# chy980959830/Multi-Modal-Retrieval-System-Image-Search-and-Data-Governance

Hardware: AMD Instinct MI355X
Metric: images/sec encode + Mqueries/sec top-10 over 1M×512 gallery, 1→8 MI355X (higher is better)
Workload: dtype bf16; 1 GPU; ViT-B/32 bf16 encode batch 256/GPU + top-10 of 256 queries over 1000000x512 bf16 gallery rows/GPU (BASELINE configs[1]); encode_batch_per_gpu=256, gallery_rows_per_gpu=1000000, gallery_rows_total=1000000, queries=256, k=10, embed_dim=512, parallelism=single GPU, launch=single process, steps_in_flight=2, weights=seeded random init (no checkpoint reachable offline)

## Files before the change

include/mmr.h:

```cpp
#ifndef MMR_H
#define MMR_H

#include <stddef.h>
#include <stdint.h>

#ifdef __cplusplus
extern "C" {
#endif

typedef enum { MMR_F32 = 0, MMR_BF16 = 1 } mmr_dtype;

enum {
    MMR_OK = 0,
    MMR_EIO = -5,
    MMR_EINVAL = -22,
    MMR_ENOSPC = -28,
    MMR_ENOTSUP = -95
};

const char *mmr_last_error(void);
int mmr_version(void);


size_t mmr_search_workspace_bytes(int64_t N, int E, int Q, int k);
// ... 109 lines not shown

typedef enum {
    MMR_P_PATCH_W = 0, MMR_P_CLS, MMR_P_POS, MMR_P_LN_PRE_W, MMR_P_LN_PRE_B,
    MMR_P_LN1_W, MMR_P_LN1_B, MMR_P_QKV_W, MMR_P_QKV_B, MMR_P_OUT_W, MMR_P_OUT_B,
    MMR_P_LN2_W, MMR_P_LN2_B, MMR_P_FC1_W, MMR_P_FC1_B, MMR_P_FC2_W, MMR_P_FC2_B,
    MMR_P_LN_FINAL_W, MMR_P_LN_FINAL_B, MMR_P_PROJ, MMR_P_TOK_EMB,
    MMR_P_TYPE_EMB,
    MMR_P_POOL_W,
    MMR_P_POOL_B,
    MMR_P_PROJ_B,
    MMR_P_QKV_C,
    MMR_P_FC1_C,
    MMR_P_COUNT
} mmr_param;

size_t mmr_tower_weights_bytes(const mmr_tower_cfg *cfg);
int mmr_tower_param_span(const mmr_tower_cfg *cfg, int param, int layer, size_t *offset, size_t *bytes);

typedef struct mmr_tower mmr_tower;

#define MMR_STATUS_BAD_TOKEN_ID 1

int mmr_tower_set_shared_chip(mmr_tower *t, int shared);
int mmr_tower_create(const mmr_tower_cfg *cfg, const void *weights, size_t weights_bytes, mmr_tower **out);
void mmr_tower_destroy(mmr_tower *t);
size_t mmr_tower_workspace_bytes(const mmr_tower *t, int batch);

int mmr_vit_encode_image(mmr_tower *t, const void *pixels, mmr_dtype in_dtype, int B, void *out,
                         mmr_dtype out_dtype, int normalize, void *workspace, size_t workspace_bytes,
                         void *stream);

int mmr_text_encode(mmr_tower *t, const int32_t *ids, int N, void *out, mmr_dtype out_dtype, int normalize,
                    void *workspace, size_t workspace_bytes, void *stream);

size_t mmr_bert_workspace_bytes(const mmr_tower *t, int N, int T);
int mmr_bert_forward(mmr_tower *t, const int32_t *ids, int N, int T, void *out, mmr_dtype out_dtype, int normalize,
                     int tap_after, float *tap, void *workspace, size_t workspace_bytes, void *stream);
int mmr_bert_forward_masked(mmr_tower *t, const int32_t *ids, const int32_t *token_type_ids,
                            const int32_t *attention_mask, int N, int T, void *out, mmr_dtype out_dtype, int normalize,
                            int tap_after, float *tap, void *workspace, size_t workspace_bytes, void *stream);

int mmr_tower_forward(mmr_tower *t, const void *input, mmr_dtype in_dtype, int B, void *out,
                      mmr_dtype out_dtype, int normalize, int tap_after, float *tap, void *workspace,
                      size_t workspace_bytes, void *stream);


// ... 44 lines not shown
```

multi-modal-retrieval-system-image-search-and-data-governance_amd/_lib.py:

```python
import ctypes
import os

import torch

_HERE = os.path.dirname(os.path.abspath(__file__))
LIB_PATH = os.environ.get("MMR_LIB") or os.path.join(_HERE, "csrc", "libmmr_hip.so")

MMR_F32, MMR_BF16 = 0, 1
_ERRNAMES = {-5: "EIO", -22: "EINVAL", -28: "ENOSPC", -95: "ENOTSUP"}


class MMRError(RuntimeError):
    def __init__(self, code, msg):
        super().__init__(f"libmmr_hip: {_ERRNAMES.get(code, code)}: {msg}")
        self.code = code


class TowerCfg(ctypes.Structure):
    _fields_ = [(n, ctypes.c_int) for n in
                ("kind", "width", "layers", "heads", "mlp", "tokens", "embed_dim", "image_size", "patch", "vocab")]
    _fields_.append(("ln_eps", ctypes.c_float))
    _fields_.append(("fold_ln", ctypes.c_int))


# ... 85 lines not shown
    L.mmr_tip_adapter_logits.argtypes = [vp, vp, vp, vp, i32, i64, i32, i32, i32, f32, f32, vp, vp, vp]
    L.mmr_preprocess_image.restype = i32
    L.mmr_preprocess_image.argtypes = [vp, i32, i32, i32, i32, i32, vp, vp, i32, vp, vp, i32, f32, f32, f32, f32, f32,
                                       f32, vp, vp, i32, vp, vp]
    L.mmr_preprocess_batch.restype = i32
    L.mmr_preprocess_batch.argtypes = [vp, i32, i32, i32, f32, f32, f32, f32, f32, f32, vp, i32, vp]
    L.mmr_preprocess_batch_ex.restype = i32
    L.mmr_preprocess_batch_ex.argtypes = [vp, i32, i32, i32, i32, f32, f32, f32, f32, f32, f32, vp, i32, vp]
    L.mmr_prof_enable.restype = i32
    L.mmr_prof_enable.argtypes = [i32, i32]
    L.mmr_prof_read.restype = i32
    L.mmr_prof_read.argtypes = [i32, ctypes.POINTER(ctypes.c_double), ctypes.POINTER(ctypes.c_longlong),
                                ctypes.POINTER(ctypes.c_longlong)]
    if hasattr(L, "mmr_tower_create"):
        cfgp = ctypes.POINTER(TowerCfg)
        L.mmr_tower_weights_bytes.restype = sz
        L.mmr_tower_weights_bytes.argtypes = [cfgp]
        L.mmr_tower_param_span.restype = i32
        L.mmr_tower_param_span.argtypes = [cfgp, i32, i32, ctypes.POINTER(sz), ctypes.POINTER(sz)]
        L.mmr_tower_create.restype = i32
        L.mmr_tower_create.argtypes = [cfgp, vp, sz, ctypes.POINTER(vp)]
        L.mmr_tower_set_shared_chip.restype = i32
        L.mmr_tower_set_shared_chip.argtypes = [vp, i32]
        L.mmr_tower_destroy.restype = None
        L.mmr_tower_destroy.argtypes = [vp]
        L.mmr_tower_workspace_bytes.restype = sz
        L.mmr_tower_workspace_bytes.argtypes = [vp, i32]
        L.mmr_vit_encode_image.restype = i32
        L.mmr_vit_encode_image.argtypes = [vp, vp, i32, i32, vp, i32, i32, vp, sz, vp]
        L.mmr_text_encode.restype = i32
        L.mmr_text_encode.argtypes = [vp, vp, i32, vp, i32, i32, vp, sz, vp]
        L.mmr_tower_forward.restype = i32
        L.mmr_tower_forward.argtypes = [vp, vp, i32, i32, vp, i32, i32, i32, vp, vp, sz, vp]
        L.mmr_bert_workspace_bytes.restype = sz
        L.mmr_bert_workspace_bytes.argtypes = [vp, i32, i32]
        L.mmr_bert_forward.restype = i32
        L.mmr_bert_forward.argtypes = [vp, vp, i32, i32, vp, i32, i32, i32, vp, vp, sz, vp]
        L.mmr_bert_forward_masked.restype = i32
        L.mmr_bert_forward_masked.argtypes = [vp, vp, vp, vp, i32, i32, vp, i32, i32, i32, vp, vp, sz, vp]
        L.mmr_debug_attention_masked.restype = i32
        L.mmr_debug_attention_masked.argtypes = [vp, vp, i32, i32, i32, vp, vp]
        L.mmr_debug_gemm.restype = i32
        L.mmr_debug_gemm.argtypes = [i32, vp, vp, i32, i32, i32, vp, vp, vp]
        L.mmr_debug_gemm_fold.restype = i32
        L.mmr_debug_gemm_fold.argtypes = [i32, vp, vp, i32, i32, i32, vp, vp, vp, vp, f32, f32, vp, vp, vp]
        L.mmr_debug_layernorm.restype = i32
# ... 44 lines not shown
```

multi-modal-retrieval-system-image-search-and-data-governance_amd/clip.py:

```python
import contextlib
import ctypes
import os
from typing import Dict, List, Optional, Union

import torch

from . import _lib
from .config import ClipConfig, TowerConfig, available_models, get_config
from .weights import make_clip_weights

_CONTEXT = 77
CLIP_MEAN = (0.48145466, 0.4578275, 0.40821073)
CLIP_STD = (0.26862954, 0.26130258, 0.27577711)


def _fold_ln_default() -> bool:
    return os.environ.get("MMR_FOLD_LN", "0") == "1"


def _tower_cfg_struct(t: TowerConfig, fold_ln: bool = False) -> _lib.TowerCfg:
    return _lib.TowerCfg(kind=0 if t.kind == "vision" else 1, width=t.width, layers=t.layers, heads=t.heads,
                         mlp=t.mlp, tokens=t.tokens, embed_dim=t.embed_dim, image_size=t.image_size,
                         patch=t.patch, vocab=t.vocab, ln_eps=t.ln_eps, fold_ln=int(bool(fold_ln)))

# ... 66 lines not shown
                put(pid, i, lw[name], bf)

        self.blob = blob.to(device)
        handle = ctypes.c_void_p()
        _lib.check(self.L.mmr_tower_create(ctypes.byref(self.c), self.blob.data_ptr(), self.blob.numel(),
                                           ctypes.byref(handle)))
        self.handle = handle
        self._lanes = {}

    def __del__(self):
        h, self.handle = getattr(self, "handle", None), None
        if h:
            try:
                self.L.mmr_tower_destroy(h)
            except Exception:
                pass

    @property
    def _ws(self):
        return self._lanes.get(0)

    def set_shared_chip(self, shared: bool) -> None:
        _lib.check(self.L.mmr_tower_set_shared_chip(self.handle, int(bool(shared))))

    def workspace(self, batch: int, lane: int = 0) -> torch.Tensor:
        need = self.L.mmr_tower_workspace_bytes(self.handle, batch)
        ws = self._lanes.get(lane)
        if ws is None or ws.numel() < need:
            ws = torch.empty(need, dtype=torch.uint8, device=self.device)
            self._lanes[lane] = ws
        return ws

    def status_word(self, lane: int = 0) -> int:
        ws = self._lanes.get(lane)
        return 0 if ws is None else int(ws[:4].view(torch.int32)[0])

    def forward(self, inp: torch.Tensor, out_dtype: torch.dtype, normalize: bool, tap_after: int = -1,
                tap: Optional[torch.Tensor] = None, out: Optional[torch.Tensor] = None, lane: int = 0) -> torch.Tensor:
        B = inp.shape[0]
        if out is None:
            out = torch.empty(B, self.cfg.embed_dim, dtype=out_dtype, device=self.device)
        elif (tuple(out.shape) != (B, self.cfg.embed_dim) or out.dtype != out_dtype or not out.is_contiguous()
              or out.device != self.device):
            raise ValueError(f"out must be a contiguous {out_dtype} [{B},{self.cfg.embed_dim}] tensor on {self.device}")
        if B == 0:
            return out
# ... 321 lines not shown
```

multi-modal-retrieval-system-image-search-and-data-governance_amd/csrc/tower.hip:

```cpp
#include "mmr_common.h"

#include <new>

namespace mmr {
enum { EPI_BIAS_BF16 = 0, EPI_BIAS_GELU_BF16 = 1, EPI_BIAS_RESID_F32 = 2, EPI_STORE_F32 = 3,
       EPI_BIAS_F32 = 4, EPI_BIAS_GELU_ERF_BF16 = 5, EPI_BIAS_TANH_BF16 = 6, EPI_LNFOLD_BF16 = 7, EPI_LNFOLD_GELU_BF16 = 8,
       EPI_RESID_STATS_F32 = 9 };
int launch_gemm(int epi, const bf16_t *A, const bf16_t *W, int M, int N, int K, const float *bias, void *out, hipStream_t st);
int launch_gemm_patch32(const bf16_t *pix, int B, int S, const bf16_t *W, int M, int N, float *out, hipStream_t st);
int launch_gemm_aux(int epi, const bf16_t *A, const bf16_t *W, int M, int N, int K, const float *bias, void *out, const GemmAux &aux, hipStream_t st);
void gemm_set_shared_chip_hint(bool on);
int launch_im2col(const void *px, mmr_dtype dt, bf16_t *ap, int B, int S, int P, int G, int K, int Kpad, hipStream_t st);
int launch_embed_vision(const float *pe, const float *cls, const float *pos, const float *lw, const float *lb, float *h, int B, int T, int d, float eps, bf16_t *xb, float2 *stats, int32_t *status, hipStream_t st);
int launch_embed_text(const int32_t *ids, const bf16_t *tok, const float *pos, float *h, int Nb, int T, int d, int vocab, bf16_t *xb, float2 *stats, int32_t *status, hipStream_t st);
int launch_layernorm(const float *h, const float *w, const float *b, bf16_t *x, int64_t rows, int d, float eps, hipStream_t st);
int launch_pool_ln(const float *h, const int32_t *ids, const float *w, const float *b, bf16_t *xc, int Nb, int T, int d, float eps, hipStream_t st);
int launch_finish(const float *feat, void *out, mmr_dtype odt, int Nb, int E, int normalize, hipStream_t st);
int launch_embed_bert(const int32_t *ids, const bf16_t *tok, const float *pos, const float *type0, const float *lw, const float *lb, float *h, bf16_t *x, int Nb, int T, int d, int vocab, float eps, const int32_t *types, int32_t *status, hipStream_t st);
int launch_layernorm_inplace(float *h, const float *w, const float *b, bf16_t *x, int64_t rows, int d, float eps, hipStream_t st);
int launch_gather_first_rows(const bf16_t *x, bf16_t *xc, int Nb, int T, int d, hipStream_t st);
int launch_attention(const bf16_t *qkv, bf16_t *o, int Bn, int T, int heads, int d, int causal, const int32_t *kmask, hipStream_t st);

static inline int round_up(int x, int a) { return (x + a - 1) / a * a; }

static int patch_k(const mmr_tower_cfg &c) { return 3 * c.patch * c.patch; }
static int patch_kpad(const mmr_tower_cfg &c) { return round_up(patch_k(c), 64); }

static const char *validate_cfg(const mmr_tower_cfg *c)
{
    if (!c) return "null config";
    if (c->kind < 0 || c->kind > 2) return "kind must be 0 (vision), 1 (text) or 2 (BERT text)";
    if (c->width != 128 && c->width != 512 && c->width != 768 && c->width != 1024) return "width must be 128, 512, 768 or 1024";
    if (c->heads * 64 != c->width) return "heads must equal width / 64 (head dim 64)";
    if (c->layers < 1 || c->layers > 64) return "layers outside [1,64]";
    if (c->mlp < 128 || c->mlp % 128) return "mlp must be a positive multiple of 128";
    if (c->embed_dim < 128 || c->embed_dim % 128) return "embed_dim must be a positive multiple of 128";
    if (c->tokens < 1 || c->tokens > 608) return "tokens outside [1,608]";
    if (!(c->ln_eps > 0.f)) return "ln_eps must be > 0";
    if (c->fold_ln != 0 && c->fold_ln != 1) return "fold_ln must be 0 or 1";
    if (c->fold_ln && c->kind == 2) return "fold_ln is for pre-LN (CLIP) towers; BERT towers are post-LN";
    if (c->kind == 0) {
        if (c->patch < 1 || c->image_size < c->patch || c->image_size % c->patch) return "image_size must be a multiple of patch";
        const int g = c->image_size / c->patch;
        if (c->tokens != 1 + g * g) return "vision tokens must equal 1 + (image_size/patch)^2";
// ... 51 lines not shown
    put(L.layer0[MMR_P_FC1_B], m * 4);
    put(L.layer0[MMR_P_FC2_W], d * m * 2);
    put(L.layer0[MMR_P_FC2_B], d * 4);
    if (c.fold_ln) {
        put(L.layer0[MMR_P_QKV_C], 3 * d * 4);
        put(L.layer0[MMR_P_FC1_C], m * 4);
    }
    L.layer_stride = off - l0;
    L.total = l0 + L.layer_stride * c.layers;
    return L;
}

static bool is_layer_param(int p) { return (p >= MMR_P_LN1_W && p <= MMR_P_FC2_B) || p == MMR_P_QKV_C || p == MMR_P_FC1_C; }

}

using namespace mmr;

struct mmr_tower {
    mmr_tower_cfg cfg;
    Layout lay;
    const char *w;
    bool shared_chip = false;
    template <typename T> const T *g(int p) const { return reinterpret_cast<const T *>(w + lay.global[p].off); }
    template <typename T> const T *l(int p, int layer) const {
        return reinterpret_cast<const T *>(w + lay.layer0[p].off + (size_t)layer * lay.layer_stride);
    }
};

extern "C" size_t mmr_tower_weights_bytes(const mmr_tower_cfg *cfg)
{
    if (validate_cfg(cfg)) return 0;
    return make_layout(*cfg).total;
}

extern "C" int mmr_tower_param_span(const mmr_tower_cfg *cfg, int param, int layer, size_t *offset, size_t *bytes)
{
    const char *why = validate_cfg(cfg);
    MMR_CHECK_ARG(!why, "mmr_tower_param_span: %s", why);
    MMR_CHECK_ARG(param >= 0 && param < MMR_P_COUNT && offset && bytes, "mmr_tower_param_span: bad param id %d", param);
    const Layout L = make_layout(*cfg);
    if (is_layer_param(param)) {
        MMR_CHECK_ARG(layer >= 0 && layer < cfg->layers, "mmr_tower_param_span: layer %d outside [0,%d)", layer, cfg->layers);
        MMR_CHECK_ARG(L.layer0[param].bytes != 0, "mmr_tower_param_span: this tower has no tensor %d", param);
        *offset = L.layer0[param].off + (size_t)layer * L.layer_stride;
        *bytes = L.layer0[param].bytes;
    } else {
        MMR_CHECK_ARG(L.global[param].bytes != 0, "mmr_tower_param_span: this tower has no tensor %d", param);
        *offset = L.global[param].off;
        *bytes = L.global[param].bytes;
    }
    return MMR_OK;
}

extern "C" int mmr_tower_create(const mmr_tower_cfg *cfg, const void *weights, size_t weights_bytes, mmr_tower **out)
{
    const char *why = validate_cfg(cfg);
    MMR_CHECK_ARG(!why, "mmr_tower_create: %s", why);
    MMR_CHECK_ARG(weights && out, "mmr_tower_create: null pointer");
    MMR_CHECK_ARG(((uintptr_t)weights & 255) == 0, "mmr_tower_create: weight blob must be 256-byte aligned");
    const Layout L = make_layout(*cfg);
    MMR_CHECK_ARG(weights_bytes >= L.total, "mmr_tower_create: blob %zu bytes < layout %zu", weights_bytes, L.total);
    mmr_tower *t = new (std::nothrow) mmr_tower;
    MMR_CHECK_ARG(t != nullptr, "mmr_tower_create: out of host memory");
    t->cfg = *cfg;
    t->lay = L;
    t->w = (const char *)weights;
    *out = t;
    return MMR_OK;
}

extern "C" void mmr_tower_destroy(mmr_tower *t) { delete t; }

namespace {
struct WsPlan {
    int M, Mpad, Mp, Mp_pad, Bpad;
    size_t off_status, off_h, off_x, off_big, off_pe, off_xc, off_feat, off_xo, off_stats, total;
};
WsPlan plan_ws(const mmr_tower_cfg &c, int B)
{
    WsPlan p{};
    p.M = B * c.tokens;
    p.Mpad = round_up(p.M, p.M >= 4096 ? 256 : 128);
    p.Bpad = round_up(B, 128);
    const size_t d = c.width;
    const size_t wide = (size_t)(c.mlp > 3 * c.width ? c.mlp : 3 * c.width);
    size_t big = (size_t)p.Mpad * wide * 2;
    size_t off = 0;
    auto put = [&](size_t &o, size_t bytes) { o = off; off += align_up(bytes, 256); };
    if (c.kind == 0) {
        p.Mp = B * (c.tokens - 1);
        p.Mp_pad = round_up(p.Mp, p.Mp >= 4096 ? 256 : 128);
        const size_t ap = (size_t)p.Mp_pad * patch_kpad(c) * 2;
        if (ap > big) big = ap;
    }
    put(p.off_status, 256);
    put(p.off_h, (size_t)p.Mpad * d * 4);
    put(p.off_x, (size_t)p.Mpad * d * 2);
    put(p.off_big, big);
    put(p.off_pe, c.kind == 0 ? (size_t)p.Mp_pad * d * 4 : 0);
    put(p.off_xc, (size_t)p.Bpad * d * 2);
    put(p.off_feat, (size_t)p.Bpad * c.embed_dim * 4);
    if (c.fold_ln) {
        put(p.off_xo, (size_t)p.Mpad * d * 2);
        put(p.off_stats, (size_t)p.Mpad * LNFOLD_NP * 8);
    }
    p.total = off;
    return p;
}
}

extern "C" int mmr_tower_set_shared_chip(mmr_tower *t, int shared)
{
    MMR_CHECK_ARG(t != nullptr, "mmr_tower_set_shared_chip: null tower");
    t->shared_chip = shared != 0;
    return MMR_OK;
}

extern "C" size_t mmr_tower_workspace_bytes(const mmr_tower *t, int batch)
{
    if (!t || batch < 1) return 0;
    return plan_ws(t->cfg, batch).total;
}

extern "C" int mmr_tower_forward(mmr_tower *t, const void *input, mmr_dtype in_dtype, int B, void *out, mmr_dtype out_dtype,
                                 int normalize, int tap_after, float *tap, void *workspace, size_t workspace_bytes,
                                 void *stream)
{
    MMR_CHECK_ARG(t != nullptr, "mmr_tower_forward: null tower");
    MMR_CHECK_ARG(t->cfg.kind != 2, "mmr_tower_forward: BERT towers run through mmr_bert_forward");
    const mmr_tower_cfg &c = t->cfg;
    MMR_CHECK_ARG(B >= 0 && B <= 65535, "mmr_tower_forward: batch %d outside [0,65535]", B);
    if (B == 0) return MMR_OK;
    MMR_CHECK_ARG(input && out && workspace, "mmr_tower_forward: null pointer");
    MMR_CHECK_ARG(out_dtype == MMR_F32 || out_dtype == MMR_BF16, "mmr_tower_forward: out dtype %d", (int)out_dtype);
    if (c.kind == 0) MMR_CHECK_ARG(in_dtype == MMR_F32 || in_dtype == MMR_BF16, "mmr_tower_forward: pixel dtype %d", (int)in_dtype);
    MMR_CHECK_ARG(((uintptr_t)input & 15) == 0 && ((uintptr_t)workspace & 255) == 0, "mmr_tower_forward: input must be 16-byte and workspace 256-byte aligned");
    MMR_CHECK_ARG(tap_after >= -1 && tap_after < c.layers, "mmr_tower_forward: tap_after %d outside [-1,%d)", tap_after, c.layers);
// ... 32 lines not shown
            rc = launch_gemm(EPI_STORE_F32, big, t->g<bf16_t>(MMR_P_PATCH_W), p.Mp_pad, d, Kp, nullptr, pe, st);
        }
        if (rc) return rc;
        if ((rc = launch_embed_vision(pe, t->g<float>(MMR_P_CLS), t->g<float>(MMR_P_POS), t->g<float>(MMR_P_LN_PRE_W),
                                      t->g<float>(MMR_P_LN_PRE_B), h, B, T, d, c.ln_eps, xb, stats, status, st))) return rc;
    } else {
        if ((rc = launch_embed_text((const int32_t *)input, t->g<bf16_t>(MMR_P_TOK_EMB), t->g<float>(MMR_P_POS), h, B, T, d,
                                    c.vocab, xb, stats, status, st))) return rc;
    }
    if (tap && tap_after == -1) MMR_CHECK_HIP(hipMemcpyAsync(tap, h, hbytes, hipMemcpyDeviceToDevice, st));

    for (int i = 0; i < c.layers && fold; ++i) {
        GemmAux a{};
        a.stats_in = stats; a.stats_out = stats; a.xout = x; a.inv_d = 1.f / (float)d; a.eps = c.ln_eps;
        a.colsum = t->l<float>(MMR_P_QKV_C, i);
        if ((rc = launch_gemm_aux(EPI_LNFOLD_BF16, x, t->l<bf16_t>(MMR_P_QKV_W, i), p.Mpad, 3 * d, d, t->l<float>(MMR_P_QKV_B, i), big, a, st))) return rc;
        if ((rc = launch_attention(big, xo, B, T, c.heads, d, c.kind == 1, nullptr, st))) return rc;
        if ((rc = launch_gemm_aux(EPI_RESID_STATS_F32, xo, t->l<bf16_t>(MMR_P_OUT_W, i), p.Mpad, d, d, t->l<float>(MMR_P_OUT_B, i), h, a, st))) return rc;
        a.colsum = t->l<float>(MMR_P_FC1_C, i);
        if ((rc = launch_gemm_aux(EPI_LNFOLD_GELU_BF16, x, t->l<bf16_t>(MMR_P_FC1_W, i), p.Mpad, m, d, t->l<float>(MMR_P_FC1_B, i), big, a, st))) return rc;
        if ((rc = launch_gemm_aux(EPI_RESID_STATS_F32, big, t->l<bf16_t>(MMR_P_FC2_W, i), p.Mpad, d, m, t->l<float>(MMR_P_FC2_B, i), h, a, st))) return rc;
        if (tap && tap_after == i) MMR_CHECK_HIP(hipMemcpyAsync(tap, h, hbytes, hipMemcpyDeviceToDevice, st));
    }
    for (int i = 0; i < c.layers && !fold; ++i) {
        if ((rc = launch_layernorm(h, t->l<float>(MMR_P_LN1_W, i), t->l<float>(MMR_P_LN1_B, i), x, p.M, d, c.ln_eps, st))) return rc;
        if ((rc = launch_gemm(EPI_BIAS_BF16, x, t->l<bf16_t>(MMR_P_QKV_W, i), p.Mpad, 3 * d, d, t->l<float>(MMR_P_QKV_B, i), big, st))) return rc;
        if ((rc = launch_attention(big, x, B, T, c.heads, d, c.kind == 1, nullptr, st))) return rc;
        if ((rc = launch_gemm(EPI_BIAS_RESID_F32, x, t->l<bf16_t>(MMR_P_OUT_W, i), p.Mpad, d, d, t->l<float>(MMR_P_OUT_B, i), h, st))) return rc;
        if ((rc = launch_layernorm(h, t->l<float>(MMR_P_LN2_W, i), t->l<float>(MMR_P_LN2_B, i), x, p.M, d, c.ln_eps, st))) return rc;
        if ((rc = launch_gemm(EPI_BIAS_GELU_BF16, x, t->l<bf16_t>(MMR_P_FC1_W, i), p.Mpad, m, d, t->l<float>(MMR_P_FC1_B, i), big, st))) return rc;
        if ((rc = launch_gemm(EPI_BIAS_RESID_F32, big, t->l<bf16_t>(MMR_P_FC2_W, i), p.Mpad, d, m, t->l<float>(MMR_P_FC2_B, i), h, st))) return rc;
        if (tap && tap_after == i) MMR_CHECK_HIP(hipMemcpyAsync(tap, h, hbytes, hipMemcpyDeviceToDevice, st));
    }

    if ((rc = launch_pool_ln(h, c.kind == 1 ? (const int32_t *)input : nullptr, t->g<float>(MMR_P_LN_FINAL_W),
                             t->g<float>(MMR_P_LN_FINAL_B), xc, B, T, d, c.ln_eps, st))) return rc;
    if ((rc = launch_gemm(EPI_STORE_F32, xc, t->g<bf16_t>(MMR_P_PROJ), p.Bpad, E, d, nullptr, feat, st))) return rc;
    return launch_finish(feat, out, out_dtype, B, E, normalize, st);
}

extern "C" int mmr_vit_encode_image(mmr_tower *t, const void *pixels, mmr_dtype in_dtype, int B, void *out,
                                    mmr_dtype out_dtype, int normalize, void *workspace, size_t workspace_bytes,
                                    void *stream)
{
    MMR_CHECK_ARG(t && t->cfg.kind == 0, "mmr_vit_encode_image: not a vision tower");
    return mmr_tower_forward(t, pixels, in_dtype, B, out, out_dtype, normalize, -1, nullptr, workspace, workspace_bytes, stream);
}

extern "C" int mmr_text_encode(mmr_tower *t, const int32_t *ids, int N, void *out, mmr_dtype out_dtype, int normalize,
                               void *workspace, size_t workspace_bytes, void *stream)
{
    MMR_CHECK_ARG(t && t->cfg.kind == 1, "mmr_text_encode: not a text tower");
    return mmr_tower_forward(t, ids, MMR_F32, N, out, out_dtype, normalize, -1, nullptr, workspace, workspace_bytes, stream);
}

namespace {
struct BertWs {
    int M, Mpad, Npad;
    size_t off_status, off_h, off_x, off_big, off_xc, off_xp, off_feat, total;
// ... 126 lines not shown
```

multi-modal-retrieval-system-image-search-and-data-governance_amd/csrc/vit_ops.hip:

```cpp
#include "mmr_common.h"

#include <math.h>

namespace mmr {

template <typename TIN>
__global__ __launch_bounds__(256) void im2col_kernel(const TIN *__restrict__ px, bf16_t *__restrict__ ap, int B,
                                                     int S, int P, int G, int K, int Kpad)
{
    const int chunks_per_row = Kpad / 8;
    const int64_t total = (int64_t)B * G * G * chunks_per_row;
    for (int64_t id = (int64_t)blockIdx.x * blockDim.x + threadIdx.x; id < total; id += (int64_t)gridDim.x * blockDim.x) {
        const int ch = (int)(id % chunks_per_row);
        const int64_t row = id / chunks_per_row;
        const int gx = (int)(row % G), gy = (int)((row / G) % G), b = (int)(row / ((int64_t)G * G));
        float v[8];
        const int k0 = ch * 8;
        if ((P & 7) == 0 && k0 + 8 <= K) {
            const int c = k0 / (P * P), rem = k0 % (P * P), ky = rem / P, kx = rem % P;
            const TIN *src = px + (((size_t)b * 3 + c) * S + (gy * P + ky)) * S + gx * P + kx;
            if constexpr (sizeof(TIN) == 4) {
                const float4 a = *reinterpret_cast<const float4 *>(src);
                const float4 bq = *reinterpret_cast<const float4 *>(src + 4);
                v[0] = a.x; v[1] = a.y; v[2] = a.z; v[3] = a.w; v[4] = bq.x; v[5] = bq.y; v[6] = bq.z; v[7] = bq.w;
// ... 178 lines not shown
    const int64_t row = (int64_t)blockIdx.x * 4 + (threadIdx.x >> 6);
    if (row >= rows) return;
    float v[VPL];
#pragma unroll
    for (int j = 0; j < VPL; ++j) v[j] = h[(size_t)row * d + j * 64 + lane];
    ln_row<VPL>(v, w, b, lane, d, eps);
#pragma unroll
    for (int j = 0; j < VPL; ++j) {
        h[(size_t)row * d + j * 64 + lane] = v[j];
        x[(size_t)row * d + j * 64 + lane] = f32_to_bf16(v[j]);
    }
}

__global__ __launch_bounds__(256) void gather_first_rows_kernel(const bf16_t *__restrict__ x, bf16_t *__restrict__ xc, int Nb,
                                                                int T, int d)
{
    const int chunks = d / 8;
    const int id = blockIdx.x * blockDim.x + threadIdx.x;
    if (id >= Nb * chunks) return;
    const int n = id / chunks, c = id % chunks;
    *reinterpret_cast<uint4 *>(xc + (size_t)n * d + c * 8) = *reinterpret_cast<const uint4 *>(x + (size_t)n * T * d + c * 8);
}

template <int VPL>
__global__ __launch_bounds__(256) void pool_ln_kernel(const float *__restrict__ h, const int32_t *__restrict__ ids,
                                                      const float *__restrict__ w, const float *__restrict__ b,
                                                      bf16_t *__restrict__ xc, int Nb, int T, int d, float eps)
{
    const int lane = threadIdx.x & 63;
    const int n = blockIdx.x * 4 + (threadIdx.x >> 6);
    if (n >= Nb) return;
    int pick = 0;
    if (ids) {
        int best = -2147483647 - 1, bpos = 0;
        for (int t = lane; t < T; t += 64) {
            const int v = ids[(size_t)n * T + t];
            if (v > best) { best = v; bpos = t; }
        }
#pragma unroll
        for (int off = 32; off >= 1; off >>= 1) {
            const int ov = __shfl_xor(best, off, 64), op = __shfl_xor(bpos, off, 64);
            if (ov > best || (ov == best && op < bpos)) { best = ov; bpos = op; }
        }
        pick = bpos;
    }
    const float *src = h + ((size_t)n * T + pick) * d;
    float v[VPL];
#pragma unroll
    for (int j = 0; j < VPL; ++j) v[j] = src[j * 64 + lane];
    ln_row<VPL>(v, w, b, lane, d, eps);
#pragma unroll
    for (int j = 0; j < VPL; ++j) xc[(size_t)n * d + j * 64 + lane] = f32_to_bf16(v[j]);
}

template <typename TOUT>
__global__ __launch_bounds__(256) void finish_kernel(const float *__restrict__ feat, TOUT *__restrict__ out, int Nb, int E,
                                                     int normalize)
{
    const int lane = threadIdx.x & 63;
    const int n = blockIdx.x * 4 + (threadIdx.x >> 6);
    if (n >= Nb) return;
    const float *f = feat + (size_t)n * E;
    float inv = 1.f;
    if (normalize) {
        float ss = 0.f;
        for (int j = lane; j < E; j += 64) ss += f[j] * f[j];
        inv = 1.0f / sqrtf(wave_sum(ss));
    }
    for (int j = lane; j < E; j += 64) {
        const float v = f[j] * inv;
        if constexpr (sizeof(TOUT) == 2) ((bf16_t *)out)[(size_t)n * E + j] = f32_to_bf16(v);
        else ((float *)out)[(size_t)n * E + j] = v;
    }
}

// ... 413 lines not shown
                    oacc[x][dt] = __builtin_amdgcn_mfma_f32_16x16x32_bf16(vf[s2][dt], pf[x].v, oacc[x][dt], 0, 0, 0);
        }
        if constexpr (!TAIL) {
            lwrite(buf ^ 1);
            __syncthreads();
        }
    };
    for (int kb = 0; kb + 1 < nkb; ++kb) block(kb, std::false_type{});
    block(nkb - 1, std::true_type{});
#pragma unroll
    for (int x = 0; x < QB; ++x) {
        const float lx = quad_rows_reduce(l[x], [](float p, float q) { return p + q; });
        const float inv = (MASKED && lx == 0.f) ? 0.f : 1.f / lx;
        const int qi = q0 + 16 * x;
        if (qi < T) {
            bf16_t *dst = o + ((size_t)b * T + qi) * d + hd * 64 + fg * 4;
#pragma unroll
            for (int dt = 0; dt < 4; ++dt) {
                uint2 pk;
                pk.x = pack_bf16x2(oacc[x][dt][0] * inv, oacc[x][dt][1] * inv);
                pk.y = pack_bf16x2(oacc[x][dt][2] * inv, oacc[x][dt][3] * inv);
                *reinterpret_cast<uint2 *>(dst + dt * 16) = pk;
            }
        }
    }
}

#define MMR_VPL_SWITCH(d, ...)                                                     \
    switch ((d) / 64) {                                                            \
        case 2: { constexpr int VPL = 2; __VA_ARGS__; } break;                     \
        case 8: { constexpr int VPL = 8; __VA_ARGS__; } break;                     \
        case 12: { constexpr int VPL = 12; __VA_ARGS__; } break;                   \
        case 16: { constexpr int VPL = 16; __VA_ARGS__; } break;                   \
        default: set_error("width %d unsupported (128, 512, 768, 1024)", (d)); return MMR_ENOTSUP; \
    }

int launch_im2col(const void *px, mmr_dtype dt, bf16_t *ap, int B, int S, int P, int G, int K, int Kpad, hipStream_t st)
{
    ProfScope prof(MMR_PROF_ROWWISE, st);
    const int64_t total = (int64_t)B * G * G * (Kpad / 8);
    const int blocks = (int)((total + 255) / 256 < 8192 ? (total + 255) / 256 : 8192);
    if (dt == MMR_F32) hipLaunchKernelGGL(im2col_kernel<float>, dim3(blocks), dim3(256), 0, st, (const float *)px, ap, B, S, P, G, K, Kpad);
    else hipLaunchKernelGGL(im2col_kernel<bf16_t>, dim3(blocks), dim3(256), 0, st, (const bf16_t *)px, ap, B, S, P, G, K, Kpad);
    MMR_CHECK_LAUNCH();
    return MMR_OK;
}
// ... 140 lines not shown
    if (kmask) {
        switch (nt) {
            case 2: return launch_attention_t<2, false, true>(qkv, o, Bn, T, heads, d, kmask, st);
            case 4: return launch_attention_t<4, false, true>(qkv, o, Bn, T, heads, d, kmask, st);
            case 6: return launch_attention_t<6, false, true>(qkv, o, Bn, T, heads, d, kmask, st);
        }
    } else if (!causal) {
        switch (nt) {
            case 2: return launch_attention_t<2, false, false>(qkv, o, Bn, T, heads, d, nullptr, st);
            case 4: return launch_attention_t<4, false, false>(qkv, o, Bn, T, heads, d, nullptr, st);
            case 6: return launch_attention_t<6, false, false>(qkv, o, Bn, T, heads, d, nullptr, st);
        }
    } else {
        switch (nt) {
            case 2: return launch_attention_t<2, true, false>(qkv, o, Bn, T, heads, d, nullptr, st);
            case 4: return launch_attention_t<4, true, false>(qkv, o, Bn, T, heads, d, nullptr, st);
            case 6: return launch_attention_t<6, true, false>(qkv, o, Bn, T, heads, d, nullptr, st);
        }
    }
    set_error("attention: %d tokens (%s) has no kernel instance", T, causal ? "causal" : "full");
    return MMR_ENOTSUP;
}

}
```

Baseline: 87690 images/s.

## Compute only the pooled token's query, attention and MLP in the final transformer block

In the last transformer layer, the change keeps K/V projections for every token but gathers the pooled token (CLS, or argmax id for text). It computes Q, attention, out-projection, LN2 and the MLP only for that one row per sample, using new pick-gather and single-query attention kernels. This removes most of the final layer's GEMM and attention work, whose other token outputs are never read after pooling. It applies only on the non-folded-LN path with large row counts, and can be disabled by environment variable or setter. It adds new kernels and workspace buffers, and the output is no longer computed by the same path as before.

```diff
diff --git a/include/mmr.h b/include/mmr.h
--- a/include/mmr.h
+++ b/include/mmr.h
@@ -155,6 +155,7 @@
 #define MMR_STATUS_BAD_TOKEN_ID 1
 
 int mmr_tower_set_shared_chip(mmr_tower *t, int shared);
+int mmr_tower_set_full_last_block(mmr_tower *t, int on);
 int mmr_tower_create(const mmr_tower_cfg *cfg, const void *weights, size_t weights_bytes, mmr_tower **out);
 void mmr_tower_destroy(mmr_tower *t);
 size_t mmr_tower_workspace_bytes(const mmr_tower *t, int batch);
diff --git a/multi-modal-retrieval-system-image-search-and-data-governance_amd/_lib.py b/multi-modal-retrieval-system-image-search-and-data-governance_amd/_lib.py
--- a/multi-modal-retrieval-system-image-search-and-data-governance_amd/_lib.py
+++ b/multi-modal-retrieval-system-image-search-and-data-governance_amd/_lib.py
@@ -131,6 +131,8 @@
         L.mmr_tower_create.argtypes = [cfgp, vp, sz, ctypes.POINTER(vp)]
         L.mmr_tower_set_shared_chip.restype = i32
         L.mmr_tower_set_shared_chip.argtypes = [vp, i32]
+        L.mmr_tower_set_full_last_block.restype = i32
+        L.mmr_tower_set_full_last_block.argtypes = [vp, i32]
         L.mmr_tower_destroy.restype = None
         L.mmr_tower_destroy.argtypes = [vp]
         L.mmr_tower_workspace_bytes.restype = sz
diff --git a/multi-modal-retrieval-system-image-search-and-data-governance_amd/clip.py b/multi-modal-retrieval-system-image-search-and-data-governance_amd/clip.py
--- a/multi-modal-retrieval-system-image-search-and-data-governance_amd/clip.py
+++ b/multi-modal-retrieval-system-image-search-and-data-governance_amd/clip.py
@@ -112,6 +112,9 @@
 
     def set_shared_chip(self, shared: bool) -> None:
         _lib.check(self.L.mmr_tower_set_shared_chip(self.handle, int(bool(shared))))
+
+    def set_full_last_block(self, on: bool) -> None:
+        _lib.check(self.L.mmr_tower_set_full_last_block(self.handle, int(bool(on))))
 
     def workspace(self, batch: int, lane: int = 0) -> torch.Tensor:
         need = self.L.mmr_tower_workspace_bytes(self.handle, batch)
diff --git a/multi-modal-retrieval-system-image-search-and-data-governance_amd/csrc/tower.hip b/multi-modal-retrieval-system-image-search-and-data-governance_amd/csrc/tower.hip
--- a/multi-modal-retrieval-system-image-search-and-data-governance_amd/csrc/tower.hip
+++ b/multi-modal-retrieval-system-image-search-and-data-governance_amd/csrc/tower.hip
@@ -1,6 +1,7 @@
 #include "mmr_common.h"
 
 #include <new>
+#include <stdlib.h>
 
 namespace mmr {
 enum { EPI_BIAS_BF16 = 0, EPI_BIAS_GELU_BF16 = 1, EPI_BIAS_RESID_F32 = 2, EPI_STORE_F32 = 3,
@@ -20,6 +21,8 @@
 int launch_layernorm_inplace(float *h, const float *w, const float *b, bf16_t *x, int64_t rows, int d, float eps, hipStream_t st);
 int launch_gather_first_rows(const bf16_t *x, bf16_t *xc, int Nb, int T, int d, hipStream_t st);
 int launch_attention(const bf16_t *qkv, bf16_t *o, int Bn, int T, int heads, int d, int causal, const int32_t *kmask, hipStream_t st);
+int launch_pick_gather(const int32_t *ids, const bf16_t *x, const float *h, bf16_t *xg, float *hc, int32_t *picks, int Nb, int T, int d, hipStream_t st);
+int launch_attention_pooled(const bf16_t *q, int ldq, const bf16_t *k, const bf16_t *v, int ldkv, const int32_t *picks, bf16_t *o, int Bn, int T, int heads, int d, int causal, hipStream_t st);
 
 static inline int round_up(int x, int a) { return (x + a - 1) / a * a; }
 
@@ -117,6 +120,7 @@
     Layout lay;
     const char *w;
     bool shared_chip = false;
+    bool full_last_block = false;
     template <typename T> const T *g(int p) const { return reinterpret_cast<const T *>(w + lay.global[p].off); }
     template <typename T> const T *l(int p, int layer) const {
         return reinterpret_cast<const T *>(w + lay.layer0[p].off + (size_t)layer * lay.layer_stride);
@@ -161,6 +165,8 @@
     t->cfg = *cfg;
     t->lay = L;
     t->w = (const char *)weights;
+    const char *full = getenv("MMR_FULL_LAST_BLOCK");
+    t->full_last_block = full && atoi(full) != 0;
     *out = t;
     return MMR_OK;
 }
@@ -171,7 +177,10 @@
 struct WsPlan {
     int M, Mpad, Mp, Mp_pad, Bpad;
     size_t off_status, off_h, off_x, off_big, off_pe, off_xc, off_feat, off_xo, off_stats, total;
+    bool pooled;
+    size_t off_picks, off_xg, off_hc, off_qc, off_oc, off_mc;
 };
+constexpr int POOLED_MIN_ROWS = 2048;
 WsPlan plan_ws(const mmr_tower_cfg &c, int B)
 {
     WsPlan p{};
@@ -200,6 +209,15 @@
         put(p.off_xo, (size_t)p.Mpad * d * 2);
         put(p.off_stats, (size_t)p.Mpad * LNFOLD_NP * 8);
     }
+    p.pooled = !c.fold_ln && p.Mpad > POOLED_MIN_ROWS;
+    if (p.pooled) {
+        put(p.off_picks, (size_t)p.Bpad * 4);
+        put(p.off_xg, (size_t)p.Bpad * d * 2);
+        put(p.off_hc, (size_t)p.Bpad * d * 4);
+        put(p.off_qc, (size_t)p.Bpad * d * 2);
+        put(p.off_oc, (size_t)p.Bpad * d * 2);
+        put(p.off_mc, (size_t)p.Bpad * c.mlp * 2);
+    }
     p.total = off;
     return p;
 }
@@ -209,6 +227,13 @@
 {
     MMR_CHECK_ARG(t != nullptr, "mmr_tower_set_shared_chip: null tower");
     t->shared_chip = shared != 0;
+    return MMR_OK;
+}
+
+extern "C" int mmr_tower_set_full_last_block(mmr_tower *t, int on)
+{
+    MMR_CHECK_ARG(t != nullptr, "mmr_tower_set_full_last_block: null tower");
+    t->full_last_block = on != 0;
     return MMR_OK;
 }
 
@@ -287,8 +312,28 @@
         if ((rc = launch_gemm_aux(EPI_RESID_STATS_F32, big, t->l<bf16_t>(MMR_P_FC2_W, i), p.Mpad, d, m, t->l<float>(MMR_P_FC2_B, i), h, a, st))) return rc;
         if (tap && tap_after == i) MMR_CHECK_HIP(hipMemcpyAsync(tap, h, hbytes, hipMemcpyDeviceToDevice, st));
     }
+    const bool pooled_last = p.pooled && !t->full_last_block && !(tap && tap_after == c.layers - 1);
+    const float *hfinal = h;
     for (int i = 0; i < c.layers && !fold; ++i) {
         if ((rc = launch_layernorm(h, t->l<float>(MMR_P_LN1_W, i), t->l<float>(MMR_P_LN1_B, i), x, p.M, d, c.ln_eps, st))) return rc;
+        if (pooled_last && i == c.layers - 1) {
+            int32_t *picks = (int32_t *)(ws + p.off_picks);
+            bf16_t *xg = (bf16_t *)(ws + p.off_xg), *qc = (bf16_t *)(ws + p.off_qc), *oc = (bf16_t *)(ws + p.off_oc);
+            bf16_t *mc = (bf16_t *)(ws + p.off_mc);
+            float *hc = (float *)(ws + p.off_hc);
+            const bf16_t *qkv_w = t->l<bf16_t>(MMR_P_QKV_W, i);
+            const float *qkv_b = t->l<float>(MMR_P_QKV_B, i);
+            if ((rc = launch_gemm(EPI_BIAS_BF16, x, qkv_w + (size_t)d * d, p.Mpad, 2 * d, d, qkv_b + d, big, st))) return rc;
+            if ((rc = launch_pick_gather(c.kind == 1 ? (const int32_t *)input : nullptr, x, h, xg, hc, picks, B, T, d, st))) return rc;
+            if ((rc = launch_gemm(EPI_BIAS_BF16, xg, qkv_w, p.Bpad, d, d, qkv_b, qc, st))) return rc;
+            if ((rc = launch_attention_pooled(qc, d, big, big + d, 2 * d, picks, oc, B, T, c.heads, d, c.kind == 1, st))) return rc;
+            if ((rc = launch_gemm(EPI_BIAS_RESID_F32, oc, t->l<bf16_t>(MMR_P_OUT_W, i), p.Bpad, d, d, t->l<float>(MMR_P_OUT_B, i), hc, st))) return rc;
+            if ((rc = launch_layernorm(hc, t->l<float>(MMR_P_LN2_W, i), t->l<float>(MMR_P_LN2_B, i), xg, B, d, c.ln_eps, st))) return rc;
+            if ((rc = launch_gemm(EPI_BIAS_GELU_BF16, xg, t->l<bf16_t>(MMR_P_FC1_W, i), p.Bpad, m, d, t->l<float>(MMR_P_FC1_B, i), mc, st))) return rc;
+            if ((rc = launch_gemm(EPI_BIAS_RESID_F32, mc, t->l<bf16_t>(MMR_P_FC2_W, i), p.Bpad, d, m, t->l<float>(MMR_P_FC2_B, i), hc, st))) return rc;
+            hfinal = hc;
+            break;
+        }
         if ((rc = launch_gemm(EPI_BIAS_BF16, x, t->l<bf16_t>(MMR_P_QKV_W, i), p.Mpad, 3 * d, d, t->l<float>(MMR_P_QKV_B, i), big, st))) return rc;
         if ((rc = launch_attention(big, x, B, T, c.heads, d, c.kind == 1, nullptr, st))) return rc;
         if ((rc = launch_gemm(EPI_BIAS_RESID_F32, x, t->l<bf16_t>(MMR_P_OUT_W, i), p.Mpad, d, d, t->l<float>(MMR_P_OUT_B, i), h, st))) return rc;
@@ -298,8 +343,13 @@
         if (tap && tap_after == i) MMR_CHECK_HIP(hipMemcpyAsync(tap, h, hbytes, hipMemcpyDeviceToDevice, st));
     }
 
-    if ((rc = launch_pool_ln(h, c.kind == 1 ? (const int32_t *)input : nullptr, t->g<float>(MMR_P_LN_FINAL_W),
-                             t->g<float>(MMR_P_LN_FINAL_B), xc, B, T, d, c.ln_eps, st))) return rc;
+    if (hfinal != h) {
+        rc = launch_pool_ln(hfinal, nullptr, t->g<float>(MMR_P_LN_FINAL_W), t->g<float>(MMR_P_LN_FINAL_B), xc, B, 1, d, c.ln_eps, st);
+    } else {
+        rc = launch_pool_ln(h, c.kind == 1 ? (const int32_t *)input : nullptr, t->g<float>(MMR_P_LN_FINAL_W),
+                            t->g<float>(MMR_P_LN_FINAL_B), xc, B, T, d, c.ln_eps, st);
+    }
+    if (rc) return rc;
     if ((rc = launch_gemm(EPI_STORE_F32, xc, t->g<bf16_t>(MMR_P_PROJ), p.Bpad, E, d, nullptr, feat, st))) return rc;
     return launch_finish(feat, out, out_dtype, B, E, normalize, st);
 }
diff --git a/multi-modal-retrieval-system-image-search-and-data-governance_amd/csrc/vit_ops.hip b/multi-modal-retrieval-system-image-search-and-data-governance_amd/csrc/vit_ops.hip
--- a/multi-modal-retrieval-system-image-search-and-data-governance_amd/csrc/vit_ops.hip
+++ b/multi-modal-retrieval-system-image-search-and-data-governance_amd/csrc/vit_ops.hip
@@ -224,6 +224,22 @@
     *reinterpret_cast<uint4 *>(xc + (size_t)n * d + c * 8) = *reinterpret_cast<const uint4 *>(x + (size_t)n * T * d + c * 8);
 }
 
+__device__ __forceinline__ int pooled_pick(const int32_t *__restrict__ ids, int n, int T, int lane)
+{
+    if (!ids) return 0;
+    int best = -2147483647 - 1, bpos = 0;
+    for (int t = lane; t < T; t += 64) {
+        const int v = ids[(size_t)n * T + t];
+        if (v > best) { best = v; bpos = t; }
+    }
+#pragma unroll
+    for (int off = 32; off >= 1; off >>= 1) {
+        const int ov = __shfl_xor(best, off, 64), op = __shfl_xor(bpos, off, 64);
+        if (ov > best || (ov == best && op < bpos)) { best = ov; bpos = op; }
+    }
+    return bpos;
+}
+
 template <int VPL>
 __global__ __launch_bounds__(256) void pool_ln_kernel(const float *__restrict__ h, const int32_t *__restrict__ ids,
                                                       const float *__restrict__ w, const float *__restrict__ b,
@@ -232,20 +248,7 @@
     const int lane = threadIdx.x & 63;
     const int n = blockIdx.x * 4 + (threadIdx.x >> 6);
     if (n >= Nb) return;
-    int pick = 0;
-    if (ids) {
-        int best = -2147483647 - 1, bpos = 0;
-        for (int t = lane; t < T; t += 64) {
-            const int v = ids[(size_t)n * T + t];
-            if (v > best) { best = v; bpos = t; }
-        }
-#pragma unroll
-        for (int off = 32; off >= 1; off >>= 1) {
-            const int ov = __shfl_xor(best, off, 64), op = __shfl_xor(bpos, off, 64);
-            if (ov > best || (ov == best && op < bpos)) { best = ov; bpos = op; }
-        }
-        pick = bpos;
-    }
+    const int pick = pooled_pick(ids, n, T, lane);
     const float *src = h + ((size_t)n * T + pick) * d;
     float v[VPL];
 #pragma unroll
@@ -253,6 +256,25 @@
     ln_row<VPL>(v, w, b, lane, d, eps);
 #pragma unroll
     for (int j = 0; j < VPL; ++j) xc[(size_t)n * d + j * 64 + lane] = f32_to_bf16(v[j]);
+}
+
+template <int VPL>
+__global__ __launch_bounds__(256) void pick_gather_kernel(const int32_t *__restrict__ ids, const bf16_t *__restrict__ x,
+                                                          const float *__restrict__ h, bf16_t *__restrict__ xg,
+                                                          float *__restrict__ hc, int32_t *__restrict__ picks, int Nb, int T,
+                                                          int d)
+{
+    const int lane = threadIdx.x & 63;
+    const int n = blockIdx.x * 4 + (threadIdx.x >> 6);
+    if (n >= Nb) return;
+    const int pick = pooled_pick(ids, n, T, lane);
+    if (lane == 0) picks[n] = pick;
+    const size_t src = ((size_t)n * T + pick) * d, dst = (size_t)n * d;
+#pragma unroll
+    for (int j = 0; j < VPL; ++j) {
+        xg[dst + j * 64 + lane] = x[src + j * 64 + lane];
+        hc[dst + j * 64 + lane] = h[src + j * 64 + lane];
+    }
 }
 
 template <typename TOUT>
@@ -712,6 +734,310 @@
                 pk.y = pack_bf16x2(oacc[x][dt][2] * inv, oacc[x][dt][3] * inv);
                 *reinterpret_cast<uint2 *>(dst + dt * 16) = pk;
             }
+        }
+    }
+}
+
+template <int NT, bool CAUSAL>
+__global__ __launch_bounds__(256) void attn_pool_kernel(const bf16_t *__restrict__ q, int ldq, const bf16_t *__restrict__ k,
+                                                        const bf16_t *__restrict__ v, int ldkv,
+                                                        const int32_t *__restrict__ picks, bf16_t *__restrict__ o, int T,
+                                                        int d, float scale, int heads, int npairs)
+{
+    constexpr int TPAD = NT * 16;
+    __shared__ __attribute__((aligned(16))) char smem[4 * TPAD * 128];
+    const int lane = threadIdx.x & 63;
+    const int wave = __builtin_amdgcn_readfirstlane(threadIdx.x >> 6);
+    const int pair = blockIdx.x * 4 + wave;
+    if (pair >= npairs) return;
+    const int b = pair / heads, hd = pair - b * heads;
+    const int qi = __builtin_amdgcn_readfirstlane(picks[b]);
+    const int qb = qi >> 4;
+    const int fr = lane & 15, fg = lane >> 4;
+    char *Vs = smem + wave * (TPAD * 128);
+    const bf16_t *kbase = k + (size_t)b * T * ldkv + hd * 64, *vbase = v + (size_t)b * T * ldkv + hd * 64;
+
+    uint4 vreg[NT * 2];
+#pragma unroll
+    for (int it = 0; it < NT * 2; ++it) {
+        vreg[it] = make_uint4(0, 0, 0, 0);
+        if (CAUSAL && ((it >> 1) & ~1) > qb) continue;
+        const int row = it * 8 + (lane >> 3);
+        vreg[it] = *reinterpret_cast<const uint4 *>(vbase + (size_t)(row < T ? row : T - 1) * ldkv + (lane & 7) * 8);
+    }
+    bf16x8 qf[2];
+#pragma unroll
+    for (int s = 0; s < 2; ++s) qf[s] = *reinterpret_cast<const bf16x8 *>(q + (size_t)b * ldq + hd * 64 + s * 32 + fg * 8);
+    bf16x8 kf[NT][2];
+#pragma unroll
+    for (int jt = 0; jt < NT; ++jt) {
+        const int row = jt * 16 + fr;
+#pragma unroll
+        for (int s = 0; s < 2; ++s) {
+            kf[jt][s] = (bf16x8){0, 0, 0, 0, 0, 0, 0, 0};
+            if (!CAUSAL || jt <= qb)
+                kf[jt][s] = *reinterpret_cast<const bf16x8 *>(kbase + (size_t)(row < T ? row : T - 1) * ldkv + (s * 4 + fg) * 8);
+        }
+    }
+#pragma unroll
+    for (int it = 0; it < NT * 2; ++it) {
+        if (CAUSAL && ((it >> 1) & ~1) > qb) continue;
+        const int row = it * 8 + (lane >> 3);
+        *reinterpret_cast<uint4 *>(Vs + row * 128 + (((lane & 7) ^ (row & 7)) << 4)) = vreg[it];
+    }
+
+    const int tq = fr >> 2, tp = fr & 3, trow = 4 * fg + tq;
+    const float c2 = scale * 1.44269504088896341f;
+    f32x4 sc[NT];
+#pragma unroll
+    for (int jt = 0; jt < NT; ++jt) {
+        f32x4 a = (f32x4){0.f, 0.f, 0.f, 0.f};
+        if (!CAUSAL || jt <= qb) {
+#pragma unroll
+            for (int s = 0; s < 2; ++s) a = __builtin_amdgcn_mfma_f32_16x16x32_bf16(kf[jt][s], qf[s], a, 0, 0, 0);
+        }
+        sc[jt] = a;
+    }
+    asm volatile("s_waitcnt lgkmcnt(0)" ::: "memory");
+    u32x2_t vraw[NT / 2][4][2];
+#pragma unroll
+    for (int s2 = 0; s2 < NT / 2; ++s2) {
+        if (CAUSAL && 2 * s2 > qb) {
+#pragma unroll
+            for (int dt = 0; dt < 4; ++dt) { vraw[s2][dt][0] = (u32x2_t){0, 0}; vraw[s2][dt][1] = (u32x2_t){0, 0}; }
+            continue;
+        }
+#pragma unroll
+        for (int dt = 0; dt < 4; ++dt) {
+            const int r0 = 32 * s2 + trow;
+            const int ch = ((dt * 2 + (tp >> 1)) ^ (trow & 7)) << 4;
+            vraw[s2][dt][0] = lds_read_tr16(Vs + r0 * 128 + ch + 8 * (tp & 1));
+            vraw[s2][dt][1] = lds_read_tr16(Vs + (r0 + 16) * 128 + ch + 8 * (tp & 1));
+        }
+    }
+    float mx = -INFINITY;
+#pragma unroll
+    for (int jt = 0; jt < NT; ++jt) {
+        if (CAUSAL && jt > qb) continue;
+#pragma unroll
+        for (int r = 0; r < 4; ++r) {
+            const int key = jt * 16 + fg * 4 + r;
+            if (key >= T || (CAUSAL && key > qi)) sc[jt][r] = -INFINITY;
+            mx = fmaxf(mx, sc[jt][r]);
+        }
+    }
+    mx = quad_rows_reduce(mx, [](float p, float q) { return fmaxf(p, q); });
+    const float m2 = mx == -INFINITY ? 0.f : mx * c2;
+    float sum = 0.f;
+#pragma unroll
+    for (int jt = 0; jt < NT; ++jt) {
+        if (CAUSAL && jt > qb) continue;
+#pragma unroll
+        for (int r = 0; r < 4; ++r) {
+            const float p = __builtin_amdgcn_exp2f(__builtin_fmaf(sc[jt][r], c2, -m2));
+            sc[jt][r] = p;
+            sum += p;
+        }
+    }
+    sum = quad_rows_reduce(sum, [](float p, float q) { return p + q; });
+    const float inv = 1.f / sum;
+
+    asm volatile("s_waitcnt lgkmcnt(0)" ::: "memory");
+#pragma unroll
+    for (int s2 = 0; s2 < NT / 2; ++s2)
+        asm volatile("" : "+v"(vraw[s2][0][0]), "+v"(vraw[s2][0][1]), "+v"(vraw[s2][1][0]), "+v"(vraw[s2][1][1]),
+                          "+v"(vraw[s2][2][0]), "+v"(vraw[s2][2][1]), "+v"(vraw[s2][3][0]), "+v"(vraw[s2][3][1]));
+    __builtin_amdgcn_sched_barrier(0);
+    f32x4 oacc[4];
+#pragma unroll
+    for (int dt = 0; dt < 4; ++dt) oacc[dt] = (f32x4){0.f, 0.f, 0.f, 0.f};
+#pragma unroll
+    for (int s2 = 0; s2 < NT / 2; ++s2) {
+        if (CAUSAL && 2 * s2 > qb) continue;
+        union { bf16x8 v; uint32_t u[4]; } pf;
+        pf.u[0] = pack_bf16x2(sc[2 * s2][0] * inv, sc[2 * s2][1] * inv);
+        pf.u[1] = pack_bf16x2(sc[2 * s2][2] * inv, sc[2 * s2][3] * inv);
+        pf.u[2] = pack_bf16x2(sc[2 * s2 + 1][0] * inv, sc[2 * s2 + 1][1] * inv);
+        pf.u[3] = pack_bf16x2(sc[2 * s2 + 1][2] * inv, sc[2 * s2 + 1][3] * inv);
+#pragma unroll
+        for (int dt = 0; dt < 4; ++dt) {
+            const bf16x8 vf = __builtin_bit_cast(bf16x8, __builtin_shufflevector(vraw[s2][dt][0], vraw[s2][dt][1], 0, 1, 2, 3));
+            oacc[dt] = __builtin_amdgcn_mfma_f32_16x16x32_bf16(vf, pf.v, oacc[dt], 0, 0, 0);
+        }
+    }
+    if (fr == 0) {
+        bf16_t *dst = o + (size_t)b * d + hd * 64 + fg * 4;
+#pragma unroll
+        for (int dt = 0; dt < 4; ++dt) {
+            uint2 pk;
+            pk.x = pack_bf16x2(oacc[dt][0], oacc[dt][1]);
+            pk.y = pack_bf16x2(oacc[dt][2], oacc[dt][3]);
+            *reinterpret_cast<uint2 *>(dst + dt * 16) = pk;
+        }
+    }
+}
+
+template <bool CAUSAL>
+__global__ __launch_bounds__(256) void attn_pool_stream_kernel(const bf16_t *__restrict__ q, int ldq,
+                                                               const bf16_t *__restrict__ k, const bf16_t *__restrict__ v,
+                                                               int ldkv, const int32_t *__restrict__ picks,
+                                                               bf16_t *__restrict__ o, int T, int d, float scale, int heads,
+                                                               int npairs)
+{
+    __shared__ __attribute__((aligned(16))) char smem[4 * AIMG];
+    const int lane = threadIdx.x & 63;
+    const int wave = __builtin_amdgcn_readfirstlane(threadIdx.x >> 6);
+    const int pair = blockIdx.x * 4 + wave;
+    if (pair >= npairs) return;
+    const int b = pair / heads, hd = pair - b * heads;
+    const int q0 = __builtin_amdgcn_readfirstlane(picks[b]);
+    const int fr = lane & 15, fg = lane >> 4;
+    char *Vs = smem + wave * AIMG;
+    const bf16_t *kbase = k + (size_t)b * T * ldkv + hd * 64, *vbase = v + (size_t)b * T * ldkv + hd * 64;
+    const int nkb = (T + AKB - 1) / AKB;
+    const float c2 = scale * 1.44269504088896341f;
+
+    bf16x8 qf[2];
+#pragma unroll
+    for (int s = 0; s < 2; ++s) qf[s] = *reinterpret_cast<const bf16x8 *>(q + (size_t)b * ldq + hd * 64 + s * 32 + fg * 8);
+
+    bf16x8 kf[4][2];
+    uint4 vreg[8];
+    auto gload = [&](int kb) {
+#pragma unroll
+        for (int jt = 0; jt < 4; ++jt) {
+            const int key = kb * AKB + jt * 16 + fr;
+#pragma unroll
+            for (int s = 0; s < 2; ++s) {
+                kf[jt][s] = (bf16x8){0, 0, 0, 0, 0, 0, 0, 0};
+                if (key < T) kf[jt][s] = *reinterpret_cast<const bf16x8 *>(kbase + (size_t)key * ldkv + (s * 4 + fg) * 8);
+            }
+        }
+#pragma unroll
+        for (int i = 0; i < 8; ++i) {
+            const int key = kb * AKB + i * 8 + (lane >> 3);
+            vreg[i] = make_uint4(0, 0, 0, 0);
+            if (key < T) vreg[i] = *reinterpret_cast<const uint4 *>(vbase + (size_t)key * ldkv + (lane & 7) * 8);
+        }
+    };
+    const int tq = fr >> 2, tp = fr & 3;
+    const int trow = 4 * fg + tq;
+
+    float m = -INFINITY, l = 0.f;
+    f32x4 oacc[4];
+#pragma unroll
+    for (int dt = 0; dt < 4; ++dt) oacc[dt] = (f32x4){0.f, 0.f, 0.f, 0.f};
+
+    gload(0);
+    auto block = [&](int kb, auto tailc) {
+        constexpr bool TAIL = decltype(tailc)::value;
+        const int njt = TAIL ? (T - kb * AKB + 15) / 16 : 4;
+#pragma unroll
+        for (int i = 0; i < 8; ++i) {
+            const int row = i * 8 + (lane >> 3);
+            *reinterpret_cast<uint4 *>(Vs + row * 128 + (((lane & 7) ^ (row & 7)) << 4)) = vreg[i];
+        }
+        f32x4 sc[4];
+#pragma unroll
+        for (int jt = 0; jt < 4; ++jt) {
+            f32x4 a = (f32x4){0.f, 0.f, 0.f, 0.f};
+            if (!TAIL || jt < njt) {
+#pragma unroll
+                for (int s = 0; s < 2; ++s) a = __builtin_amdgcn_mfma_f32_16x16x32_bf16(kf[jt][s], qf[s], a, 0, 0, 0);
+            }
+            sc[jt] = a;
+        }
+        if constexpr (!TAIL) gload(kb + 1);
+        asm volatile("s_waitcnt lgkmcnt(0)" ::: "memory");
+        u32x2_t vraw[2][4][2];
+#pragma unroll
+        for (int s2 = 0; s2 < 2; ++s2) {
+            if (TAIL && 2 * s2 >= njt) {
+#pragma unroll
+                for (int dt = 0; dt < 4; ++dt) { vraw[s2][dt][0] = (u32x2_t){0, 0}; vraw[s2][dt][1] = (u32x2_t){0, 0}; }
+                continue;
+            }
+#pragma unroll
+            for (int dt = 0; dt < 4; ++dt) {
+                const int r0 = 32 * s2 + trow;
+                const int ch = ((dt * 2 + (tp >> 1)) ^ (trow & 7)) << 4;
+                vraw[s2][dt][0] = lds_read_tr16(Vs + r0 * 128 + ch + 8 * (tp & 1));
+                vraw[s2][dt][1] = lds_read_tr16(Vs + (r0 + 16) * 128 + ch + 8 * (tp & 1));
+            }
+        }
+        if (CAUSAL || TAIL) {
+#pragma unroll
+            for (int jt = 0; jt < 4; ++jt) {
+                if (TAIL && jt >= njt) continue;
+#pragma unroll
+                for (int r = 0; r < 4; ++r) {
+                    const int key = kb * AKB + jt * 16 + fg * 4 + r;
+                    if (key >= T || (CAUSAL && key > q0)) sc[jt][r] = -INFINITY;
+                }
+            }
+        }
+        float bm = fmaxf(fmaxf(sc[0][0], sc[0][1]), fmaxf(sc[0][2], sc[0][3]));
+#pragma unroll
+        for (int jt = 1; jt < 4; ++jt)
+            if (!TAIL || jt < njt)
+                bm = fmaxf(bm, fmaxf(fmaxf(sc[jt][0], sc[jt][1]), fmaxf(sc[jt][2], sc[jt][3])));
+        bm = quad_rows_reduce(bm, [](float p, float q) { return fmaxf(p, q); });
+        const float mn = fmaxf(m, bm * c2);
+        const float msafe = mn == -INFINITY ? 0.f : mn;
+        const bool moved = mn != m;
+        const float alpha = __builtin_amdgcn_exp2f(m - msafe);
+        m = mn;
+        float ps = 0.f;
+#pragma unroll
+        for (int jt = 0; jt < 4; ++jt) {
+            if (TAIL && jt >= njt) continue;
+#pragma unroll
+            for (int r = 0; r < 4; ++r) {
+                const float p = __builtin_amdgcn_exp2f(__builtin_fmaf(sc[jt][r], c2, -msafe));
+                sc[jt][r] = p;
+                ps += p;
+            }
+        }
+        l = l * alpha + ps;
+        if (__any(moved)) {
+#pragma unroll
+            for (int dt = 0; dt < 4; ++dt)
+#pragma unroll
+                for (int r = 0; r < 4; ++r) oacc[dt][r] *= alpha;
+        }
+        asm volatile("s_waitcnt lgkmcnt(0)" ::: "memory");
+#pragma unroll
+        for (int s2 = 0; s2 < 2; ++s2)
+            asm volatile("" : "+v"(vraw[s2][0][0]), "+v"(vraw[s2][0][1]), "+v"(vraw[s2][1][0]), "+v"(vraw[s2][1][1]),
+                              "+v"(vraw[s2][2][0]), "+v"(vraw[s2][2][1]), "+v"(vraw[s2][3][0]), "+v"(vraw[s2][3][1]));
+        __builtin_amdgcn_sched_barrier(0);
+#pragma unroll
+        for (int s2 = 0; s2 < 2; ++s2) {
+            if (TAIL && 2 * s2 >= njt) continue;
+            union { bf16x8 v; uint32_t u[4]; } pf;
+            pf.u[0] = pack_bf16x2(sc[2 * s2][0], sc[2 * s2][1]);
+            pf.u[1] = pack_bf16x2(sc[2 * s2][2], sc[2 * s2][3]);
+            pf.u[2] = pack_bf16x2(sc[2 * s2 + 1][0], sc[2 * s2 + 1][1]);
+            pf.u[3] = pack_bf16x2(sc[2 * s2 + 1][2], sc[2 * s2 + 1][3]);
+#pragma unroll
+            for (int dt = 0; dt < 4; ++dt) {
+                const bf16x8 vf = __builtin_bit_cast(bf16x8, __builtin_shufflevector(vraw[s2][dt][0], vraw[s2][dt][1], 0, 1, 2, 3));
+                oacc[dt] = __builtin_amdgcn_mfma_f32_16x16x32_bf16(vf, pf.v, oacc[dt], 0, 0, 0);
+            }
+        }
+    };
+    for (int kb = 0; kb + 1 < nkb; ++kb) block(kb, std::false_type{});
+    block(nkb - 1, std::true_type{});
+    const float lx = quad_rows_reduce(l, [](float p, float q) { return p + q; });
+    const float inv = 1.f / lx;
+    if (fr == 0) {
+        bf16_t *dst = o + (size_t)b * d + hd * 64 + fg * 4;
+#pragma unroll
+        for (int dt = 0; dt < 4; ++dt) {
+            uint2 pk;
+            pk.x = pack_bf16x2(oacc[dt][0] * inv, oacc[dt][1] * inv);
+            pk.y = pack_bf16x2(oacc[dt][2] * inv, oacc[dt][3] * inv);
+            *reinterpret_cast<uint2 *>(dst + dt * 16) = pk;
         }
     }
 }
@@ -898,4 +1224,32 @@
     return MMR_ENOTSUP;
 }
 
-}
+int launch_pick_gather(const int32_t *ids, const bf16_t *x, const float *h, bf16_t *xg, float *hc, int32_t *picks, int Nb, int T,
+                       int d, hipStream_t st)
+{
+    ProfScope prof(MMR_PROF_ROWWISE, st);
+    const dim3 grid((unsigned)((Nb + 3) / 4));
+    MMR_VPL_SWITCH(d, hipLaunchKernelGGL(pick_gather_kernel<VPL>, grid, dim3(256), 0, st, ids, x, h, xg, hc, picks, Nb, T, d));
+    MMR_CHECK_LAUNCH();
+    return MMR_OK;
+}
+
+int launch_attention_pooled(const bf16_t *q, int ldq, const bf16_t *k, const bf16_t *v, int ldkv, const int32_t *picks, bf16_t *o,
+                            int Bn, int T, int heads, int d, int causal, hipStream_t st)
+{
+    ProfScope prof(MMR_PROF_ATTENTION, st);
+    const int npairs = heads * Bn;
+    const dim3 grid((unsigned)((npairs + 3) / 4));
+#define MMR_POOL_ATT(...) hipLaunchKernelGGL((__VA_ARGS__), grid, dim3(256), 0, st, q, ldq, k, v, ldkv, picks, o, T, d, 0.125f, heads, npairs)
+    switch ((T + 31) / 32 * 2) {
+        case 2: if (causal) MMR_POOL_ATT(attn_pool_kernel<2, true>); else MMR_POOL_ATT(attn_pool_kernel<2, false>); break;
+        case 4: if (causal) MMR_POOL_ATT(attn_pool_kernel<4, true>); else MMR_POOL_ATT(attn_pool_kernel<4, false>); break;
+        case 6: if (causal) MMR_POOL_ATT(attn_pool_kernel<6, true>); else MMR_POOL_ATT(attn_pool_kernel<6, false>); break;
+        default: if (causal) MMR_POOL_ATT(attn_pool_stream_kernel<true>); else MMR_POOL_ATT(attn_pool_stream_kernel<false>); break;
+    }
+#undef MMR_POOL_ATT
+    MMR_CHECK_LAUNCH();
+    return MMR_OK;
+}
+
+}
```

After: 93980 images/s (median of 6 runs). 1.07x the previous value.
